# BadgerTechnologies/navigation

Measured on AMD Instinct MI355X. Metric: scored trajectories/sec (whole node) + costmap inflation cells/sec, 400x400 map, higher is better.
Workload: dtype f64

## Files before the change

### include/navgpu.h

```cpp
#ifndef NAVGPU_H_
#define NAVGPU_H_

#include <stddef.h>
#include <stdint.h>

#ifdef __cplusplus
extern "C" {
#endif

typedef enum {
  NAVGPU_OK = 0,
  NAVGPU_ERR_INVALID = -1,
  NAVGPU_ERR_NO_DEVICE = -2,
  NAVGPU_ERR_HIP = -3,
  NAVGPU_ERR_CAPACITY = -4,
  NAVGPU_ERR_STATE = -5
} navgpu_status;

#define NAVGPU_NO_INFORMATION 255
#define NAVGPU_LETHAL_OBSTACLE 254
#define NAVGPU_INSCRIBED_INFLATED_OBSTACLE 253
#define NAVGPU_FREE_SPACE 0

#define NAVGPU_LAYER_STATIC 1
// ... 177 lines not shown
  double acc_lim_x, acc_lim_y, acc_lim_theta;
  double xy_goal_tolerance, yaw_goal_tolerance;
  double trans_stopped_vel, rot_stopped_vel;
  int32_t prune_plan, reserved;
} navgpu_robot_limits;
int navgpu_planner_set_limits(navgpu_fleet* fleet, uint32_t first, uint32_t count, const navgpu_robot_limits* limits);
int navgpu_planner_get_limits(navgpu_fleet* fleet, uint32_t first, uint32_t count, navgpu_robot_limits* limits);
int navgpu_planner_set_plan(navgpu_fleet* fleet, uint32_t first, uint32_t count);
int navgpu_planner_stage(navgpu_fleet* fleet, uint32_t first, uint32_t count, const navgpu_robot_state* states,
                         const double* plan_xy, uint32_t n_plan_total);
int navgpu_planner_stage_poses(navgpu_fleet* fleet, uint32_t first, uint32_t count, const float* pos_xyth, const float* vel_xyth);
int navgpu_planner_cycle(navgpu_fleet* fleet, uint32_t first, uint32_t count);
int navgpu_planner_set_bounded_map_grids(navgpu_fleet* fleet, int32_t enable);
int navgpu_planner_set_seed_lists(navgpu_fleet* fleet, int32_t enable);
int navgpu_planner_set_split_prep(navgpu_fleet* fleet, int32_t enable);
int navgpu_planner_set_seed_list_capacity(navgpu_fleet* fleet, uint32_t cells);
int navgpu_planner_seed_list_counts(navgpu_fleet* fleet, uint32_t first, uint32_t count, uint32_t* counts);
int navgpu_planner_set_map_grid_options(navgpu_fleet* fleet, int32_t critic, int32_t aggregation, double yshift);
int navgpu_planner_wavefront_levels(navgpu_fleet* fleet, uint32_t first, uint32_t count, uint32_t* levels);
int navgpu_planner_wavefront_boxes(navgpu_fleet* fleet, uint32_t first, uint32_t count, int32_t* boxes);
int navgpu_planner_results(navgpu_fleet* fleet, uint32_t first, uint32_t count, navgpu_plan_result* results);
int navgpu_planner_set_cycles_in_flight(navgpu_fleet* fleet, int32_t cycles);
int navgpu_planner_results_previous(navgpu_fleet* fleet, uint32_t first, uint32_t count, navgpu_plan_result* results);
int navgpu_planner_trajectory(navgpu_fleet* fleet, uint32_t instance, double* xyth, uint32_t capacity_points);
int navgpu_planner_samples(navgpu_fleet* fleet, uint32_t instance, double* costs, int32_t* status,
                           float* velocities_xyz, uint32_t capacity);
int navgpu_planner_check_trajectory(navgpu_fleet* fleet, uint32_t instance, const float vel_samples[3], int32_t* ok);
int navgpu_planner_check_trajectories(navgpu_fleet* fleet, uint32_t n_robots, const uint32_t* instances,
                                      const uint32_t* probe_offsets , const float* vel_samples ,
                                      int32_t* ok , double* costs );
// ... 595 lines not shown
```

### navigation_amd/_lib.py

```python
import ctypes as C
import os
import subprocess

import numpy as np

_HERE = os.path.dirname(os.path.abspath(__file__))
_LIB = None

LAYER_STATIC, LAYER_OBSTACLE, LAYER_VOXEL, LAYER_INFLATION = 1, 2, 4, 8
GRID_MASTER, GRID_STATIC, GRID_OBSTACLE, GRID_VOXEL, GRID_PATH, GRID_GOAL, GRID_GOAL_FRONT = range(7)
OBS_MARKING, OBS_CLEARING = 1, 2
VOXEL_UNKNOWN, VOXEL_MARKED = 1, 2
K_OBSTACLE, K_MERGE, K_INFLATE, K_BFS, K_SCORE, K_SELECT, K_FOOTPRINT, K_VOXEL_EXPORT, K_OBS_INGEST, K_CHECK_TRAJ = range(10)
KERNELS = ("k_obstacle", "k_merge", "k_inflate", "k_bfs", "k_score", "k_select", "k_footprint_cost", "k_voxel_export", "k_obs_ingest", "k_check_traj")
CLOUD_XYZ, CLOUD_SCAN = 0, 1
OBSBUF_MAX_SOURCES, OBSBUF_MAX_CLOUD_POINTS = 8, 65536


class NavgpuError(RuntimeError):
    pass


class FleetDesc(C.Structure):
    _fields_ = [("n_instances", C.c_uint32), ("size_x", C.c_uint32), ("size_y", C.c_uint32),
# ... 439 lines not shown
    ("navgpu_costmap_update_list", C.c_int, [vp, u32, vp]),
    ("navgpu_costmap_bounds_list", C.c_int, [vp, u32, vp, vp]),
    ("navgpu_inflate", C.c_int, [vp, u32, u32, vp]),
    ("navgpu_obstacle_update_bounds", C.c_int, [vp, u32, u32, vp]),
    ("navgpu_obstacle_update_costs", C.c_int, [vp, u32, u32, vp]),
    ("navgpu_planner_configure", C.c_int, [vp, C.POINTER(DwaConfig)]),
    ("navgpu_planner_set_limits", C.c_int, [vp, C.c_uint32, C.c_uint32, vp]),
    ("navgpu_planner_get_limits", C.c_int, [vp, C.c_uint32, C.c_uint32, vp]),
    ("navgpu_planner_set_plan", C.c_int, [vp, u32, u32]),
    ("navgpu_planner_stage", C.c_int, [vp, u32, u32, vp, vp, u32]),
    ("navgpu_planner_stage_poses", C.c_int, [vp, u32, u32, vp, vp]),
    ("navgpu_planner_cycle", C.c_int, [vp, u32, u32]),
    ("navgpu_planner_set_bounded_map_grids", C.c_int, [vp, C.c_int32]),
    ("navgpu_planner_set_seed_lists", C.c_int, [vp, C.c_int32]),
    ("navgpu_planner_set_split_prep", C.c_int, [vp, C.c_int32]),
    ("navgpu_planner_set_seed_list_capacity", C.c_int, [vp, u32]),
    ("navgpu_planner_seed_list_counts", C.c_int, [vp, u32, u32, vp]),
    ("navgpu_planner_set_map_grid_options", C.c_int, [vp, C.c_int32, C.c_int32, C.c_double]),
    ("navgpu_planner_wavefront_levels", C.c_int, [vp, u32, u32, vp]),
    ("navgpu_planner_wavefront_boxes", C.c_int, [vp, u32, u32, vp]),
    ("navgpu_planner_results", C.c_int, [vp, u32, u32, vp]),
    ("navgpu_planner_set_cycles_in_flight", C.c_int, [vp, C.c_int32]),
    ("navgpu_planner_results_previous", C.c_int, [vp, u32, u32, vp]),
    ("navgpu_planner_trajectory", C.c_int, [vp, u32, vp, u32]),
    ("navgpu_planner_samples", C.c_int, [vp, u32, vp, vp, vp, u32]),
    ("navgpu_planner_check_trajectory", C.c_int, [vp, u32, vp, C.POINTER(i32)]),
    ("navgpu_planner_check_trajectories", C.c_int, [vp, u32, vp, vp, vp, vp, vp]),
    ("navgpu_planner_stage_list", C.c_int, [vp, u32, vp, vp, vp, u32]),
    ("navgpu_planner_stage_poses_list", C.c_int, [vp, u32, vp, vp, vp]),
    ("navgpu_planner_cycle_list", C.c_int, [vp, u32, vp]),
# ... 151 lines not shown
```

### navigation_amd/csrc/navgpu_device.h

```cpp
#pragma once
#include <hip/hip_runtime.h>
#include <stdint.h>

#include "../../include/navgpu.h"

namespace navgpu {

constexpr uint8_t kNoInfo = 255, kLethal = 254, kInscribed = 253, kFree = 0;
constexpr int kMaxFootprint = 32;
constexpr int kCareRows = 128, kCareWords = 4;
constexpr uint32_t kSeedListMax = 1024;
constexpr uint32_t kNoSeedList = 0xFFFFFFFFu;
#ifndef NAVGPU_SCORE_TAB_THREADS
#define NAVGPU_SCORE_TAB_THREADS 256
#endif
#ifndef NAVGPU_SCORE_TAB_LDS_KB
#define NAVGPU_SCORE_TAB_LDS_KB 14
#endif
#ifndef NAVGPU_SCORE_PREP_THREADS
#define NAVGPU_SCORE_PREP_THREADS 256
#endif
#ifndef NAVGPU_SCORE_THREADS
#define NAVGPU_SCORE_THREADS 256
#endif
// ... 111 lines not shown
  int32_t* axis_count;
  uint32_t *path, *goal, *goal_front;
  uint32_t* bfs_scratch;
  int32_t* bfs_box;
  uint32_t* bfs_care;
  uint32_t* bfs_reach;
  uint32_t bfs_bounded;
  unsigned long long* bfs_trace;
  uint32_t* bfs_next_item;
  uint32_t* bfs_free;
  uint32_t* bfs_levels;
  uint32_t* bfs_order;
  uint32_t* bfs_seed_cells;
  uint32_t* bfs_seed_count;
  uint32_t bfs_seed_cap;
  uint32_t bfs_grids;
  uint32_t* within;
  uint32_t win;
  uint32_t fp_rcells;
  uint8_t fp_halfw[32];
  uint32_t fp_chunk;
  uint32_t use_tables, tab_steps, tab_nfp, tab_nth;
  int32_t mg_agg[4];
  double mg_yshift[4];
  int32_t mg_generic;
  uint32_t tab_rows;
  uint32_t tab_bytes;
  double tab_dt;
  uint8_t* prep;
  uint32_t prep_stride, prep_bytes;
// ... 410 lines not shown
```

### navigation_amd/csrc/navgpu_fleet.h

```cpp
#pragma once
#include <algorithm>
#include <cfloat>
#include <cmath>
#include <cstdio>
#include <cstdlib>
#include <cstring>
#include <ctime>
#include <deque>
#include <mutex>
#include <string>
#include <vector>

#include "navgpu_device.h"

using namespace navgpu;

namespace navgpu {
extern thread_local std::string g_last_error;

#define HIP_TRY(expr)                                                                              \
  do {                                                                                             \
    hipError_t e_ = (expr);                                                                        \
    if (e_ != hipSuccess) {                                                                        \
      g_last_error = std::string(#expr) + ": " + hipGetErrorString(e_);                            \
// ... 45 lines not shown
  navgpu_inflation_params infl{};
  navgpu_obstacle_params obsp{};
  double fp_radius = 0.0;
  std::vector<void*> pinned;
  ObsCsr* hp_obs = nullptr;
  uint32_t *hp_cnt = nullptr, *hp_used = nullptr, *hp_plan_cnt = nullptr;
  float* hp_pts = nullptr;
  double *hp_fpw = nullptr, *hp_pose = nullptr, *hp_plan = nullptr, *hp_front = nullptr;
  int32_t *hp_shift = nullptr, *hp_align = nullptr;
  uint32_t *hp_reach = nullptr, *hp_fpn = nullptr;
  uint8_t *cm_stage_dev = nullptr, *cm_stage_host = nullptr, *pl_stage_dev = nullptr, *pl_stage_host = nullptr;
  size_t cm_stage_bytes = 0, pl_stage_bytes = 0;
  bool bounded_grids = true;
  bool seed_lists = true;
  bool split_prep = true;
  uint32_t seed_list_cap = kSeedListMax;
  std::vector<uint8_t> grid_partial;
  std::vector<int32_t> h_box;
  std::vector<uint64_t> inputs_gen, cycle_gen;
  void touchInputs(uint32_t first, uint32_t count) {
    for (uint32_t i = first; i < first + count && i < inputs_gen.size(); ++i) ++inputs_gen[i];
  }
  navgpu_robot_state* hp_state = nullptr;
  navgpu_plan_result* hp_result = nullptr;
  bool hp_dma_pending = false;
  int cycles_in_flight = 1;
  int res_slot = 0;
  hipEvent_t ev_cycle[2] = {nullptr, nullptr}, ev_cm_h2d = nullptr, ev_pl_h2d = nullptr;
  bool ev_cycle_set[2] = {false, false}, ev_cm_set = false, ev_pl_set = false;
  hipError_t waitMirrors(hipEvent_t ev, bool set) {
// ... 286 lines not shown
```

### navigation_amd/csrc/navgpu_host.cpp

```cpp
#include "navgpu_fleet.h"

namespace navgpu {
thread_local std::string g_last_error;
}

extern "C" {

const char* navgpu_version(void) { return "navgpu 0.1 (gfx950)"; }
const char* navgpu_strerror(int status) {
  switch (status) {
    case NAVGPU_OK: return "ok";
    case NAVGPU_ERR_INVALID: return "invalid argument";
    case NAVGPU_ERR_NO_DEVICE: return "no usable HIP device (this library has no CPU fallback)";
    case NAVGPU_ERR_HIP: return "HIP runtime error";
    case NAVGPU_ERR_CAPACITY: return "input exceeds a capacity given at fleet creation";
    case NAVGPU_ERR_STATE: return "call sequence violated";
    default: return "unknown status";
  }
}
const char* navgpu_last_error(void) { return g_last_error.c_str(); }
int navgpu_device_count(void) {
  int n = 0;
  if (hipGetDeviceCount(&n) != hipSuccess) return 0;
  return n;
// ... 184 lines not shown
  A(pl.goal, (size_t)n * pl.cells);
  A(pl.goal_front, (size_t)n * pl.cells);
  if (bfs_scratch_words(cm.nx, cm.ny)) A(pl.bfs_scratch, (size_t)n * bfs_scratch_words(cm.nx, cm.ny));
  pl.bfs_grids = 3;
  pl.within = nullptr;
  A(pl.bfs_box, (size_t)n * 8);
  A(pl.bfs_care, (size_t)n * kCareRows * kCareWords);
  A(pl.bfs_next_item, 4);
  A(pl.bfs_free, (size_t)n * cm.ny * ((cm.nx + 31) / 32));
  A(pl.bfs_levels, (size_t)n * 3);
  A(pl.bfs_order, (size_t)n * 3);
  A(pl.bfs_seed_cells, (size_t)n * 3 * kSeedListMax);
  A(pl.bfs_seed_count, (size_t)n * 3);
  pl.bfs_seed_cap = 0;
  pl.bfs_bounded = 0;
  A(pl.counters, (size_t)n * 2);
  A(pl.osc_flags, n);
  A(pl.osc_prev, (size_t)n * 3);
  A(pl.limits, n);
  A(pl.traj, (size_t)n * pl.max_sim_steps * 3);
#undef A
  f->h_origin.assign((size_t)n * 2, 0.0);
  f->h_fp_spec.assign((size_t)n * kMaxFootprint * 2, 0.0);
  f->h_fp_n.assign(n, 0);
  f->h_limits.assign(n, RobotLimits{});
  f->limits_dirty.assign(n, 0);
  f->lp_lim.assign(n, navgpu_local_limits{});
  f->grid_partial.assign(n, 0);
  f->obs_consumed.assign(n, 0);
  f->bounded_grids = true;
// ... 919 lines not shown
  if (!f) return NAVGPU_ERR_INVALID;
  FleetGuard guard_(f);
  f->bounded_grids = enable != 0;
  return restageReach(f);
}
int navgpu_planner_set_seed_lists(navgpu_fleet* f, int32_t enable) {
  if (!f) return NAVGPU_ERR_INVALID;
  FleetGuard guard_(f);
  f->seed_lists = enable != 0;
  return NAVGPU_OK;
}
int navgpu_planner_set_split_prep(navgpu_fleet* f, int32_t enable) {
  if (!f) return NAVGPU_ERR_INVALID;
  FleetGuard guard_(f);
  f->split_prep = enable != 0;
  return NAVGPU_OK;
}
static bool splitPrep(const navgpu_fleet* f) {
  return f->split_prep && split_prep_applies && launch_bfs_prep && launch_bfs_prep_list && launch_score_grids && launch_score_grids_list &&
         split_prep_applies(f->pl);
}
int navgpu_planner_set_seed_list_capacity(navgpu_fleet* f, uint32_t cells) {
  if (!f || cells == 0 || cells > kSeedListMax) return NAVGPU_ERR_INVALID;
  FleetGuard guard_(f);
  f->seed_list_cap = cells;
  return NAVGPU_OK;
}
int navgpu_planner_seed_list_counts(navgpu_fleet* f, uint32_t first, uint32_t count, uint32_t* counts) {
  if (!f || !counts || !f->rangeOk(first, count)) return NAVGPU_ERR_INVALID;
  FleetGuard guard_(f);
// ... 868 lines not shown
```

### navigation_amd/csrc/planner_bfs_rows.hip

```cpp
#include "planner_bfs_common.h"
#include "planner_score.h"

namespace navgpu {

#ifdef NAVGPU_BFS_STATS
__device__ unsigned long long g_bfs_stats[16];
#define BFS_STAMP(v) const unsigned long long v = __builtin_amdgcn_s_memtime()
#define BFS_ACC(i, x) bst[i] += (x)
#else
#define BFS_STAMP(v)
#define BFS_ACC(i, x)
#endif
#ifndef NAVGPU_ROWS_RECORD_PAD
#define NAVGPU_ROWS_RECORD_PAD 4
#endif
constexpr uint32_t kRowsRecordPad = NAVGPU_ROWS_RECORD_PAD;
template <int W>
__host__ __device__ inline size_t bfs_rows_lds_words(uint32_t nx, uint32_t ny) {
  constexpr uint32_t Wp = (W + 3) & ~3u;
  const uint32_t nw = bfs_rows_waves(ny);
  return (((size_t)nw * kRowsPerWave * ((nx + 31) >> 5) + 3) & ~(size_t)3) + (size_t)kCareRows * kCareWords + (size_t)(nw + 2) * 2 * kRowsHalo * (2 * Wp + kRowsRecordPad);
}
#define NAVGPU_ROWS_DPP " row_mask:0xf bank_mask:0xf bound_ctrl:1\n\t"
#define NAVGPU_ROWS_GROUP_WORDS                                    \
// ... 16 lines not shown
  "v_or_b32_dpp %[t1], %[f1], %[t1] wave_shl:1" NAVGPU_ROWS_DPP    \
  "v_or_b32_dpp %[t2], %[f2], %[t2] wave_shl:1" NAVGPU_ROWS_DPP    \
  "v_or_b32_dpp %[t3], %[f3], %[t3] wave_shl:1" NAVGPU_ROWS_DPP    \
  "v_bitop3_b32 %[f0], %[u0], %[b0], %[t0] bitop3:0x32\n\t"        \
  "v_bitop3_b32 %[f1], %[u1], %[b1], %[t1] bitop3:0x32\n\t"        \
  "v_bitop3_b32 %[f2], %[u2], %[b2], %[t2] bitop3:0x32\n\t"        \
  "v_bitop3_b32 %[f3], %[u3], %[b3], %[t3] bitop3:0x32\n\t"        \
  "v_or3_b32 %[b0], %[b0], %[u0], %[t0]\n\t"                       \
  "v_or3_b32 %[b1], %[b1], %[u1], %[t1]\n\t"                       \
  "v_or3_b32 %[b2], %[b2], %[u2], %[t2]\n\t"                       \
  "v_or3_b32 %[b3], %[b3], %[u3], %[t3]\n\t"
#define NAVGPU_ROWS_GROUP_REGS                                                                                                              \
  [b0] "+v"(b[0]), [b1] "+v"(b[1]), [b2] "+v"(b[2]), [b3] "+v"(b[3]), [f0] "+v"(f[0]), [f1] "+v"(f[1]), [f2] "+v"(f[2]), [f3] "+v"(f[3]), \
      [p] "=&v"(p), [u0] "=&v"(u0), [u1] "=&v"(u1), [u2] "=&v"(u2), [u3] "=&v"(u3), [t0] "=&v"(t0), [t1] "=&v"(t1), [t2] "=&v"(t2),       \
      [t3] "=&v"(t3)
__device__ __forceinline__ void rowsGroup4(const int g, const uint32_t aw, uint64_t& acc, uint32_t* __restrict__ b, uint32_t* __restrict__ f,
                                           const uint32_t L, const uint32_t R, uint32_t& p) {
  uint32_t u0, u1, u2, u3, t0, t1, t2, t3;
  uint64_t c0;
  asm volatile(NAVGPU_ROWS_GROUP_WORDS
               "v_or3_b32 %[u0], %[f0], %[f1], %[f2]\n\t"
               "v_or_b32_e32 %[u0], %[u0], %[f3]\n\t"
               "v_cmp_ne_u32_e64 %[c0], 0, %[u0]\n\t"
               "s_or_b64 %[acc], %[acc], %[c0]\n\t"
               "1:\n\t"
               : NAVGPU_ROWS_GROUP_REGS, [acc] "+s"(acc), [c0] "=&s"(c0)
               : [aw] "s"(aw), [g] "n"(g), [L] "v"(L), [R] "v"(R)
               : "scc");
}
__device__ __forceinline__ void rowsGroup4PerLevel(const int g, const uint32_t aw, uint32_t& nz, uint32_t& lo, uint32_t& hi, uint32_t* __restrict__ b,
                                                   uint32_t* __restrict__ f, const uint32_t L, const uint32_t R, uint32_t& p) {
  uint32_t u0, u1, u2, u3, t0, t1, t2, t3, st;
  uint64_t c0, c1, c2;
  asm volatile(NAVGPU_ROWS_GROUP_WORDS
               "v_or3_b32 %[u0], %[f0], %[f1], %[f2]\n\t"
               "v_cmp_ne_u32_e64 %[c1], 0, %[f0]\n\t"
               "v_or_b32_e32 %[u0], %[u0], %[f3]\n\t"
               "v_cmp_ne_u32_e64 %[c2], 0, %[f3]\n\t"
               "v_cmp_ne_u32_e64 %[c0], 0, %[u0]\n\t"
               "s_cmp_lg_u64 %[c1], 0\n\t"
               "s_cselect_b32 %[st], %[bit], 0\n\t"
               "s_or_b32 %[lo], %[lo], %[st]\n\t"
               "s_cmp_lg_u64 %[c2], 0\n\t"
               "s_cselect_b32 %[st], %[bit], 0\n\t"
// ... 81 lines not shown
  const bool wave_in_box = (int)(wave_id * kRowsPerWave) <= by1 && (int)((wave_id + 1) * kRowsPerWave) > by0;
  const bool row_in_box = owner && row_i >= by0 && row_i <= by1;
  const int w0 = rg.w0, w1 = rg.w1;
  const uint32_t region_groups = bfsRegionGroups(rg);
  uint32_t* drow = dist + (size_t)row * nx;
  auto storeCells = [&](int j, uint32_t cells, uint32_t value) { bfsStoreCells(drow + j * 32, cells, value, aligned4); };
  const bool pub_top = lane >= (uint32_t)D && lane < 2u * D, pub_bot = lane >= 64u - 2 * D && lane < 64u - D;
  const uint32_t pub_wr = (((wave_id + 1) * 2 + (pub_top ? 0u : 1u)) * D + (pub_top ? lane - D : lane - (64u - 2 * D))) * RS;
  const bool halo_top = lane < (uint32_t)D, halo_bot = lane >= 64u - D;
  const uint32_t halo_rd = ((halo_top ? (wave_id * 2 + 1) : ((wave_id + 2) * 2)) * D + (halo_top ? lane : lane - (64u - D))) * RS;
  constexpr uint32_t gmask = (1u << NG) - 1u;

  constexpr bool kBlockLive = W != 20;
  static_assert(D >= 1 && D < 32, "the edge masks take D bits of one word");
  constexpr uint32_t edge_lo = kBlockLive ? (1u << D) - 1u : 0xFFFFFFFFu, edge_hi = kBlockLive ? ~(0xFFFFFFFFu >> D) : 0xFFFFFFFFu;
  auto activity = [&]() -> uint32_t {
    uint32_t nz = 0, lo = 0, hi = 0;
#pragma unroll
    for (int q = 0; q < NG; ++q) {
      const uint32_t t = fr[4 * q] | fr[4 * q + 1] | fr[4 * q + 2] | fr[4 * q + 3];
      if (__builtin_amdgcn_ballot_w64(t != 0) != 0) {
        nz |= 1u << q;
        if (__builtin_amdgcn_ballot_w64((fr[4 * q] & edge_lo) != 0) != 0) lo |= 1u << q;
        if (__builtin_amdgcn_ballot_w64((fr[4 * q + 3] & edge_hi) != 0) != 0) hi |= 1u << q;
      }
    }
    return (nz | (lo >> 1) | (hi << 1)) & gmask;
  };
  if (wave_in_box) {
#pragma unroll
    for (int j = 0; j < W; ++j)
      if (j >= w0 && j <= w1 && row_in_box) storeCells(j, fr[j], 0u);
  }
  uint32_t a_own = activity();
  uint32_t level = 0, xch = 0;
  bfsStamp(pl, tid, item, 2);
  bool done = false;
#ifdef NAVGPU_BFS_STATS
  unsigned long long bst[9] = {0, 0, 0, 0, 0, 0, 0, 0, 0};
#endif
  auto storeNew = [&](const uint32_t groups) {
    if (wave_in_box && (groups & region_groups) != 0) {
#pragma unroll
      for (int q = 0; q < NG; ++q) {
        if (((groups & region_groups) >> q) & 1u) {
#pragma unroll
          for (int c = 0; c < 4; ++c) {
            const int j = 4 * q + c;
            if (j < W && j >= w0 && j <= w1) {
#ifndef NAVGPU_BFS_X_NOSTORE
              if (row_in_box && fr[j < W ? j : 0] != 0) storeCells(j, fr[j < W ? j : 0], level + 1);
#endif
            }
          }
        }
      }
    }
  };
  while (!done) {
    bool any_new;
    if constexpr (kBlockLive) {
      const uint32_t aw = __builtin_amdgcn_readfirstlane(a_own);
      uint64_t acc = 0;
      if (aw == 0) {
        BFS_ACC(5, D);
        level += D;
      } else {
        for (int k = 0; k < D; ++k) {
          BFS_STAMP(ts1);
          BFS_ACC(5, 1);
          BFS_ACC(7, 1);
          BFS_ACC(8, __builtin_popcount(aw));
          uint32_t awk = aw;
          asm volatile("" : "+s"(awk));
          uint32_t p[2];
          const uint32_t zero = 0;
#pragma unroll
          for (int q = 0; q < NG; ++q)
            rowsGroup4(q, awk, acc, &blocked[4 * q], &fr[4 * q], q > 0 ? p[(q + 1) & 1] : zero, q + 1 < NG ? fr[q + 1 < NG ? 4 * q + 4 : 0] : zero, p[q & 1]);
          BFS_STAMP(ts2);
          BFS_ACC(1, ts2 - ts1);
          storeNew(awk);
          BFS_STAMP(ts3);
          BFS_ACC(2, ts3 - ts2);
          ++level;
        }
      }
      any_new = acc != 0;
    } else {
      uint32_t any_blk = 0;
      for (int k = 0; k < D; ++k) {
        BFS_STAMP(ts1);
        BFS_ACC(5, 1);
        const uint32_t aw = __builtin_amdgcn_readfirstlane(a_own);
// ... 67 lines not shown
          blocked[q] = b.x;
          blocked[q + 1] = b.y;
          blocked[q + 2] = b.z;
          blocked[q + 3] = b.w;
        }
      }
      a_own = activity();
      __syncthreads();
    }
    ++xch;
    BFS_STAMP(ts6);
    BFS_ACC(4, ts6 - ts5);
  }
#ifdef NAVGPU_BFS_STATS
  if (lane == 0)
    for (int k = 0; k < 9; ++k) atomicAdd(&g_bfs_stats[k], bst[k]);
#endif
  bfsStamp(pl, tid, item, 3);

  __syncthreads();
  {
    uint32_t ex[WP], fb[WP];
#pragma unroll
    for (int j = 0; j < WP; ++j) {
      const bool in = owner && (uint32_t)j < Wr;
      fb[j] = in ? (freew[row * Wr + j] & ((uint32_t)j + 1 == Wr ? last_mask : 0xFFFFFFFFu)) : 0u;
      ex[j] = in ? ((blocked[j] & fb[j]) | seedm[row * Wr + j]) : 0u;
    }
    if (pub_top || pub_bot) {
#pragma unroll
      for (int j = 0; j < WP; ++j) edge[pub_wr + j] = ex[j];
// ... 275 lines not shown
    return (nz | (lo >> 1) | (hi << 1)) & gmask;
  };
  if (wave_in_box) {
#pragma unroll
    for (int j = 0; j < W; ++j)
      if (j >= w0 && j <= w1) {
        if (inA) storeCells(rowA, j, frA[j], 0u);
        if (inB) storeCells(rowB, j, frB[j], 0u);
      }
  }
  uint32_t a_own = activity();
  uint32_t level = 0, xch = 0;
  bfsStamp(pl, tid, item, 2);
  bool done = false;
#ifdef NAVGPU_BFS_STATS
  unsigned long long bst[9] = {0, 0, 0, 0, 0, 0, 0, 0, 0};
#endif
  while (!done) {
    const uint32_t aw = __builtin_amdgcn_readfirstlane(a_own);
    uint64_t acc = 0;
    for (int k = 0; k < D; ++k) {
      BFS_STAMP(ts1);
      BFS_ACC(5, 1);
      uint32_t awk = aw;
      asm volatile("" : "+s"(awk));
      BFS_ACC(7, awk != 0 ? 1 : 0);
      BFS_ACC(8, __builtin_popcount(awk));
      if (awk == 0) {
        ++level;
        continue;
      }
// ... 247 lines not shown
```

### navigation_amd/fleet.py

```python
import ctypes as C

import numpy as np

from . import _lib as N
from ._lib import (DwaConfig, FleetDesc, InflationParams, NavgpuError, Observation, ObstacleParams, PlanResult,
                   RobotState, check, lib)

_GRID_DTYPE = {N.GRID_MASTER: np.uint8, N.GRID_STATIC: np.uint8, N.GRID_OBSTACLE: np.uint8,
               N.GRID_VOXEL: np.uint32, N.GRID_PATH: np.uint32, N.GRID_GOAL: np.uint32,
               N.GRID_GOAL_FRONT: np.uint32}


def _ptr(a):
    return a.ctypes.data_as(C.c_void_p)


class Fleet:
    def __init__(self, n_instances, size_x, size_y, resolution, layers=N.LAYER_OBSTACLE | N.LAYER_INFLATION,
                 track_unknown=False, device=0, max_points=1024, max_observations=4, max_plan=256,
                 max_footprint=16, max_sim_steps=64, keep_sample_costs=False, rolling_window=False):
        self.L = lib()
        d = FleetDesc(n_instances, size_x, size_y, resolution, layers, int(track_unknown), device, max_points,
                      max_observations, max_plan, max_footprint, max_sim_steps, int(keep_sample_costs), int(rolling_window))
        self.desc = d
# ... 374 lines not shown
    AGGREGATIONS = {"last": 0, "sum": 1, "product": 2}

    def set_map_grid_options(self, critic, aggregation="last", yshift=0.0):
        check(self.L.navgpu_planner_set_map_grid_options(self.h, self.MAP_GRID_CRITICS[critic], self.AGGREGATIONS[aggregation], float(yshift)),
              "set_map_grid_options")

    def set_bounded_map_grids(self, enable):
        check(self.L.navgpu_planner_set_bounded_map_grids(self.h, 1 if enable else 0), "set_bounded_map_grids")

    def set_seed_lists(self, enable):
        check(self.L.navgpu_planner_set_seed_lists(self.h, 1 if enable else 0), "set_seed_lists")

    def set_split_prep(self, enable):
        check(self.L.navgpu_planner_set_split_prep(self.h, 1 if enable else 0), "set_split_prep")

    def set_seed_list_capacity(self, cells):
        check(self.L.navgpu_planner_set_seed_list_capacity(self.h, int(cells)), "set_seed_list_capacity")

    def seed_list_counts(self, first=0, count=None):
        first, count = self._range(first, count)
        out = np.zeros((count, 3), np.uint32)
        check(self.L.navgpu_planner_seed_list_counts(self.h, first, count, _ptr(out)), "seed_list_counts")
        return out

    def wavefront_levels(self, first=0, count=None):
        first, count = self._range(first, count)
        out = np.zeros((count, 3), np.uint32)
        check(self.L.navgpu_planner_wavefront_levels(self.h, first, count, _ptr(out)), "wavefront_levels")
        return out

# ... 450 lines not shown
```

Before: 6.867 billion.

## Restrict row-bitset BFS levels to a five-word live window per wave

Adds a word-window mode to the row-bitset BFS. When the activity mask is computed, each word is checked for frontier reach, and the start of a five-word window that covers every live word is encoded into the upper bits of the activity value. Each level then updates only those five words through hand-written inline assembly, and falls back to the per-group path when no window fits. This is meant to cut the ALU/DPP work per BFS level on sparse frontiers, at the price of an extra liveness scan per activity check and larger branchy asm blocks. It is enabled by default through a new fleet flag.

```diff
diff --git a/include/navgpu.h b/include/navgpu.h
--- a/include/navgpu.h
+++ b/include/navgpu.h
@@ -215,6 +215,7 @@
 int navgpu_planner_set_bounded_map_grids(navgpu_fleet* fleet, int32_t enable);
 int navgpu_planner_set_seed_lists(navgpu_fleet* fleet, int32_t enable);
 int navgpu_planner_set_split_prep(navgpu_fleet* fleet, int32_t enable);
+int navgpu_planner_set_bfs_word_window(navgpu_fleet* fleet, int32_t enable);
 int navgpu_planner_set_seed_list_capacity(navgpu_fleet* fleet, uint32_t cells);
 int navgpu_planner_seed_list_counts(navgpu_fleet* fleet, uint32_t first, uint32_t count, uint32_t* counts);
 int navgpu_planner_set_map_grid_options(navgpu_fleet* fleet, int32_t critic, int32_t aggregation, double yshift);
diff --git a/navigation_amd/_lib.py b/navigation_amd/_lib.py
--- a/navigation_amd/_lib.py
+++ b/navigation_amd/_lib.py
@@ -477,6 +477,7 @@
     ("navgpu_planner_set_bounded_map_grids", C.c_int, [vp, C.c_int32]),
     ("navgpu_planner_set_seed_lists", C.c_int, [vp, C.c_int32]),
     ("navgpu_planner_set_split_prep", C.c_int, [vp, C.c_int32]),
+    ("navgpu_planner_set_bfs_word_window", C.c_int, [vp, C.c_int32]),
     ("navgpu_planner_set_seed_list_capacity", C.c_int, [vp, u32]),
     ("navgpu_planner_seed_list_counts", C.c_int, [vp, u32, u32, vp]),
     ("navgpu_planner_set_map_grid_options", C.c_int, [vp, C.c_int32, C.c_int32, C.c_double]),
diff --git a/navigation_amd/csrc/navgpu_device.h b/navigation_amd/csrc/navgpu_device.h
--- a/navigation_amd/csrc/navgpu_device.h
+++ b/navigation_amd/csrc/navgpu_device.h
@@ -149,6 +149,7 @@
   uint32_t* bfs_seed_cells;
   uint32_t* bfs_seed_count;
   uint32_t bfs_seed_cap;
+  uint32_t bfs_word_window;
   uint32_t bfs_grids;
   uint32_t* within;
   uint32_t win;
diff --git a/navigation_amd/csrc/navgpu_fleet.h b/navigation_amd/csrc/navgpu_fleet.h
--- a/navigation_amd/csrc/navgpu_fleet.h
+++ b/navigation_amd/csrc/navgpu_fleet.h
@@ -83,6 +83,7 @@
   bool bounded_grids = true;
   bool seed_lists = true;
   bool split_prep = true;
+  bool bfs_word_window = true;
   uint32_t seed_list_cap = kSeedListMax;
   std::vector<uint8_t> grid_partial;
   std::vector<int32_t> h_box;
diff --git a/navigation_amd/csrc/navgpu_host.cpp b/navigation_amd/csrc/navgpu_host.cpp
--- a/navigation_amd/csrc/navgpu_host.cpp
+++ b/navigation_amd/csrc/navgpu_host.cpp
@@ -222,6 +222,7 @@
   A(pl.bfs_seed_count, (size_t)n * 3);
   pl.bfs_seed_cap = 0;
   pl.bfs_bounded = 0;
+  pl.bfs_word_window = f->bfs_word_window ? 1u : 0u;
   A(pl.counters, (size_t)n * 2);
   A(pl.osc_flags, n);
   A(pl.osc_prev, (size_t)n * 3);
@@ -1171,6 +1172,13 @@
   if (!f) return NAVGPU_ERR_INVALID;
   FleetGuard guard_(f);
   f->split_prep = enable != 0;
+  return NAVGPU_OK;
+}
+int navgpu_planner_set_bfs_word_window(navgpu_fleet* f, int32_t enable) {
+  if (!f) return NAVGPU_ERR_INVALID;
+  FleetGuard guard_(f);
+  f->bfs_word_window = enable != 0;
+  f->pl.bfs_word_window = enable != 0 ? 1u : 0u;
   return NAVGPU_OK;
 }
 static bool splitPrep(const navgpu_fleet* f) {
diff --git a/navigation_amd/csrc/planner_bfs_rows.hip b/navigation_amd/csrc/planner_bfs_rows.hip
--- a/navigation_amd/csrc/planner_bfs_rows.hip
+++ b/navigation_amd/csrc/planner_bfs_rows.hip
@@ -1,4 +1,5 @@
 #include "planner_bfs_common.h"
+#include "planner_bfs_window.h"
 #include "planner_score.h"
 
 namespace navgpu {
@@ -54,20 +55,225 @@
   [b0] "+v"(b[0]), [b1] "+v"(b[1]), [b2] "+v"(b[2]), [b3] "+v"(b[3]), [f0] "+v"(f[0]), [f1] "+v"(f[1]), [f2] "+v"(f[2]), [f3] "+v"(f[3]), \
       [p] "=&v"(p), [u0] "=&v"(u0), [u1] "=&v"(u1), [u2] "=&v"(u2), [u3] "=&v"(u3), [t0] "=&v"(t0), [t1] "=&v"(t1), [t2] "=&v"(t2),       \
       [t3] "=&v"(t3)
-__device__ __forceinline__ void rowsGroup4(const int g, const uint32_t aw, uint64_t& acc, uint32_t* __restrict__ b, uint32_t* __restrict__ f,
-                                           const uint32_t L, const uint32_t R, uint32_t& p) {
-  uint32_t u0, u1, u2, u3, t0, t1, t2, t3;
+#define NAVGPU_F(i) "%[f" #i "]"
+#define NAVGPU_B(i) "%[b" #i "]"
+#define NAVGPU_ROWS_LEVEL_WINDOW(Lw, a, b, c, d, e, Rw)                                                   \
+  "v_alignbit_b32 %[u0], " NAVGPU_F(a) ", " Lw ", 31\n\t"                                                 \
+  "v_alignbit_b32 %[u1], " NAVGPU_F(b) ", " NAVGPU_F(a) ", 31\n\t"                                        \
+  "v_alignbit_b32 %[u2], " NAVGPU_F(c) ", " NAVGPU_F(b) ", 31\n\t"                                        \
+  "v_alignbit_b32 %[u3], " NAVGPU_F(d) ", " NAVGPU_F(c) ", 31\n\t"                                        \
+  "v_alignbit_b32 %[u4], " NAVGPU_F(e) ", " NAVGPU_F(d) ", 31\n\t"                                        \
+  "v_alignbit_b32 %[t0], " NAVGPU_F(b) ", " NAVGPU_F(a) ", 1\n\t"                                         \
+  "v_alignbit_b32 %[t1], " NAVGPU_F(c) ", " NAVGPU_F(b) ", 1\n\t"                                         \
+  "v_alignbit_b32 %[t2], " NAVGPU_F(d) ", " NAVGPU_F(c) ", 1\n\t"                                         \
+  "v_alignbit_b32 %[t3], " NAVGPU_F(e) ", " NAVGPU_F(d) ", 1\n\t"                                         \
+  "v_alignbit_b32 %[t4], " Rw ", " NAVGPU_F(e) ", 1\n\t"                                                  \
+  "v_or_b32_dpp %[u0], " NAVGPU_F(a) ", %[u0] wave_shr:1" NAVGPU_ROWS_DPP                                 \
+  "v_or_b32_dpp %[u1], " NAVGPU_F(b) ", %[u1] wave_shr:1" NAVGPU_ROWS_DPP                                 \
+  "v_or_b32_dpp %[u2], " NAVGPU_F(c) ", %[u2] wave_shr:1" NAVGPU_ROWS_DPP                                 \
+  "v_or_b32_dpp %[u3], " NAVGPU_F(d) ", %[u3] wave_shr:1" NAVGPU_ROWS_DPP                                 \
+  "v_or_b32_dpp %[u4], " NAVGPU_F(e) ", %[u4] wave_shr:1" NAVGPU_ROWS_DPP                                 \
+  "v_or_b32_dpp %[t0], " NAVGPU_F(a) ", %[t0] wave_shl:1" NAVGPU_ROWS_DPP                                 \
+  "v_or_b32_dpp %[t1], " NAVGPU_F(b) ", %[t1] wave_shl:1" NAVGPU_ROWS_DPP                                 \
+  "v_or_b32_dpp %[t2], " NAVGPU_F(c) ", %[t2] wave_shl:1" NAVGPU_ROWS_DPP                                 \
+  "v_or_b32_dpp %[t3], " NAVGPU_F(d) ", %[t3] wave_shl:1" NAVGPU_ROWS_DPP                                 \
+  "v_or_b32_dpp %[t4], " NAVGPU_F(e) ", %[t4] wave_shl:1" NAVGPU_ROWS_DPP                                 \
+  "v_bitop3_b32 " NAVGPU_F(a) ", %[u0], " NAVGPU_B(a) ", %[t0] bitop3:0x32\n\t"                           \
+  "v_bitop3_b32 " NAVGPU_F(b) ", %[u1], " NAVGPU_B(b) ", %[t1] bitop3:0x32\n\t"                           \
+  "v_bitop3_b32 " NAVGPU_F(c) ", %[u2], " NAVGPU_B(c) ", %[t2] bitop3:0x32\n\t"                           \
+  "v_bitop3_b32 " NAVGPU_F(d) ", %[u3], " NAVGPU_B(d) ", %[t3] bitop3:0x32\n\t"                           \
+  "v_bitop3_b32 " NAVGPU_F(e) ", %[u4], " NAVGPU_B(e) ", %[t4] bitop3:0x32\n\t"                           \
+  "v_or3_b32 " NAVGPU_B(a) ", " NAVGPU_B(a) ", %[u0], %[t0]\n\t"                                          \
+  "v_or3_b32 " NAVGPU_B(b) ", " NAVGPU_B(b) ", %[u1], %[t1]\n\t"                                          \
+  "v_or3_b32 " NAVGPU_B(c) ", " NAVGPU_B(c) ", %[u2], %[t2]\n\t"                                          \
+  "v_or3_b32 " NAVGPU_B(d) ", " NAVGPU_B(d) ", %[u3], %[t3]\n\t"                                          \
+  "v_or3_b32 " NAVGPU_B(e) ", " NAVGPU_B(e) ", %[u4], %[t4]\n\t"                                          \
+  "v_or3_b32 %[u0], " NAVGPU_F(a) ", " NAVGPU_F(b) ", " NAVGPU_F(c) "\n\t"                                \
+  "v_or3_b32 %[u0], %[u0], " NAVGPU_F(d) ", " NAVGPU_F(e) "\n\t"                                          \
+  "v_cmp_ne_u32_e64 %[c0], 0, %[u0]\n\t"                                                                  \
+  "s_or_b64 %[acc], %[acc], %[c0]\n\t"
+#define NAVGPU_ROWS_LEVEL_GROUP(g, Lw, a, b, c, d, Rw, P)                                                 \
+  "v_mov_b32 " P ", " NAVGPU_F(d) "\n\t"                                                                  \
+  "s_bitcmp1_b32 %[aw], " #g "\n\t"                                                                       \
+  "s_cbranch_scc0 1f\n\t"                                                                                 \
+  "v_alignbit_b32 %[u0], " NAVGPU_F(a) ", " Lw ", 31\n\t"                                                 \
+  "v_alignbit_b32 %[u1], " NAVGPU_F(b) ", " NAVGPU_F(a) ", 31\n\t"                                        \
+  "v_alignbit_b32 %[u2], " NAVGPU_F(c) ", " NAVGPU_F(b) ", 31\n\t"                                        \
+  "v_alignbit_b32 %[u3], " NAVGPU_F(d) ", " NAVGPU_F(c) ", 31\n\t"                                        \
+  "v_alignbit_b32 %[t0], " NAVGPU_F(b) ", " NAVGPU_F(a) ", 1\n\t"                                         \
+  "v_alignbit_b32 %[t1], " NAVGPU_F(c) ", " NAVGPU_F(b) ", 1\n\t"                                         \
+  "v_alignbit_b32 %[t2], " NAVGPU_F(d) ", " NAVGPU_F(c) ", 1\n\t"                                         \
+  "v_alignbit_b32 %[t3], " Rw ", " NAVGPU_F(d) ", 1\n\t"                                                  \
+  "v_or_b32_dpp %[u0], " NAVGPU_F(a) ", %[u0] wave_shr:1" NAVGPU_ROWS_DPP                                 \
+  "v_or_b32_dpp %[u1], " NAVGPU_F(b) ", %[u1] wave_shr:1" NAVGPU_ROWS_DPP                                 \
+  "v_or_b32_dpp %[u2], " NAVGPU_F(c) ", %[u2] wave_shr:1" NAVGPU_ROWS_DPP                                 \
+  "v_or_b32_dpp %[u3], " NAVGPU_F(d) ", %[u3] wave_shr:1" NAVGPU_ROWS_DPP                                 \
+  "v_or_b32_dpp %[t0], " NAVGPU_F(a) ", %[t0] wave_shl:1" NAVGPU_ROWS_DPP                                 \
+  "v_or_b32_dpp %[t1], " NAVGPU_F(b) ", %[t1] wave_shl:1" NAVGPU_ROWS_DPP                                 \
+  "v_or_b32_dpp %[t2], " NAVGPU_F(c) ", %[t2] wave_shl:1" NAVGPU_ROWS_DPP                                 \
+  "v_or_b32_dpp %[t3], " NAVGPU_F(d) ", %[t3] wave_shl:1" NAVGPU_ROWS_DPP                                 \
+  "v_bitop3_b32 " NAVGPU_F(a) ", %[u0], " NAVGPU_B(a) ", %[t0] bitop3:0x32\n\t"                           \
+  "v_bitop3_b32 " NAVGPU_F(b) ", %[u1], " NAVGPU_B(b) ", %[t1] bitop3:0x32\n\t"                           \
+  "v_bitop3_b32 " NAVGPU_F(c) ", %[u2], " NAVGPU_B(c) ", %[t2] bitop3:0x32\n\t"                           \
+  "v_bitop3_b32 " NAVGPU_F(d) ", %[u3], " NAVGPU_B(d) ", %[t3] bitop3:0x32\n\t"                           \
+  "v_or3_b32 " NAVGPU_B(a) ", " NAVGPU_B(a) ", %[u0], %[t0]\n\t"                                          \
+  "v_or3_b32 " NAVGPU_B(b) ", " NAVGPU_B(b) ", %[u1], %[t1]\n\t"                                          \
+  "v_or3_b32 " NAVGPU_B(c) ", " NAVGPU_B(c) ", %[u2], %[t2]\n\t"                                          \
+  "v_or3_b32 " NAVGPU_B(d) ", " NAVGPU_B(d) ", %[u3], %[t3]\n\t"                                          \
+  "v_or3_b32 %[u0], " NAVGPU_F(a) ", " NAVGPU_F(b) ", " NAVGPU_F(c) "\n\t"                                \
+  "v_or_b32_e32 %[u0], %[u0], " NAVGPU_F(d) "\n\t"                                                        \
+  "v_cmp_ne_u32_e64 %[c0], 0, %[u0]\n\t"                                                                  \
+  "s_or_b64 %[acc], %[acc], %[c0]\n\t"                                                                    \
+  "1:\n\t"
+#define NAVGPU_ROWS_LEVEL_REGS8                                                                                                             \
+  [b0] "+v"(b[0]), [b1] "+v"(b[1]), [b2] "+v"(b[2]), [b3] "+v"(b[3]), [b4] "+v"(b[4]), [b5] "+v"(b[5]), [b6] "+v"(b[6]), [b7] "+v"(b[7]), \
+      [f0] "+v"(f[0]), [f1] "+v"(f[1]), [f2] "+v"(f[2]), [f3] "+v"(f[3]), [f4] "+v"(f[4]), [f5] "+v"(f[5]), [f6] "+v"(f[6]), [f7] "+v"(f[7])
+#define NAVGPU_ROWS_LEVEL_REGS16                                                                                                                     \
+  NAVGPU_ROWS_LEVEL_REGS8, [b8] "+v"(b[8]), [b9] "+v"(b[9]), [b10] "+v"(b[10]), [b11] "+v"(b[11]), [b12] "+v"(b[12]), [b13] "+v"(b[13]),             \
+      [b14] "+v"(b[14]), [b15] "+v"(b[15]), [f8] "+v"(f[8]), [f9] "+v"(f[9]), [f10] "+v"(f[10]), [f11] "+v"(f[11]), [f12] "+v"(f[12]), [f13] "+v"(f[13]), \
+      [f14] "+v"(f[14]), [f15] "+v"(f[15])
+#define NAVGPU_ROWS_LEVEL_TEMPS                                                                                                              \
+  [u0] "=&v"(u0), [u1] "=&v"(u1), [u2] "=&v"(u2), [u3] "=&v"(u3), [u4] "=&v"(u4), [t0] "=&v"(t0), [t1] "=&v"(t1), [t2] "=&v"(t2), [t3] "=&v"(t3), \
+      [t4] "=&v"(t4), [acc] "+s"(acc), [c0] "=&s"(c0)
+static_assert(kRowsWindow == 5, "NAVGPU_ROWS_LEVEL_WINDOW is written out for five words");
+template <int W>
+__device__ __forceinline__ void rowsLevel(const uint32_t aw, uint64_t& acc, uint32_t* __restrict__ b, uint32_t* __restrict__ f) {
+  static_assert(W == 7 || W == 13, "one statement per row size, its words and windows written out");
+  uint32_t u0, u1, u2, u3, u4, t0, t1, t2, t3, t4;
   uint64_t c0;
-  asm volatile(NAVGPU_ROWS_GROUP_WORDS
-               "v_or3_b32 %[u0], %[f0], %[f1], %[f2]\n\t"
-               "v_or_b32_e32 %[u0], %[u0], %[f3]\n\t"
-               "v_cmp_ne_u32_e64 %[c0], 0, %[u0]\n\t"
-               "s_or_b64 %[acc], %[acc], %[c0]\n\t"
-               "1:\n\t"
-               : NAVGPU_ROWS_GROUP_REGS, [acc] "+s"(acc), [c0] "=&s"(c0)
-               : [aw] "s"(aw), [g] "n"(g), [L] "v"(L), [R] "v"(R)
-               : "scc");
-}
+  if constexpr (W == 7) {
+    asm volatile("s_bitcmp1_b32 %[aw], 9\n\t"
+                 "s_cbranch_scc1 12f\n\t"
+                 "s_bitcmp1_b32 %[aw], 8\n\t"
+                 "s_cbranch_scc0 20f\n\t"
+                 NAVGPU_ROWS_LEVEL_WINDOW(NAVGPU_F(0), 1, 2, 3, 4, 5, NAVGPU_F(6))
+                 "s_branch 9f\n\t"
+                 "20:\n\t"
+                 NAVGPU_ROWS_LEVEL_WINDOW("0", 0, 1, 2, 3, 4, NAVGPU_F(5))
+                 "s_branch 9f\n\t"
+                 "12:\n\t"
+                 "s_bitcmp1_b32 %[aw], 8\n\t"
+                 "s_cbranch_scc0 22f\n\t"
+                 NAVGPU_ROWS_LEVEL_GROUP(0, "0", 0, 1, 2, 3, NAVGPU_F(4), "%[u4]")
+                 NAVGPU_ROWS_LEVEL_GROUP(1, "%[u4]", 4, 5, 6, 7, "0", "%[t4]")
+                 "s_branch 9f\n\t"
+                 "22:\n\t"
+                 NAVGPU_ROWS_LEVEL_WINDOW(NAVGPU_F(1), 2, 3, 4, 5, 6, NAVGPU_F(7))
+                 "9:\n\t"
+                 : NAVGPU_ROWS_LEVEL_REGS8, NAVGPU_ROWS_LEVEL_TEMPS
+                 : [aw] "s"(aw)
+                 : "scc");
+  } else {
+    asm volatile("s_bitcmp1_b32 %[aw], 11\n\t"
+                 "s_cbranch_scc1 18f\n\t"
+                 "s_bitcmp1_b32 %[aw], 10\n\t"
+                 "s_cbranch_scc1 14f\n\t"
+                 "s_bitcmp1_b32 %[aw], 9\n\t"
+                 "s_cbranch_scc1 12f\n\t"
+                 "s_bitcmp1_b32 %[aw], 8\n\t"
+                 "s_cbranch_scc0 20f\n\t"
+                 NAVGPU_ROWS_LEVEL_WINDOW(NAVGPU_F(0), 1, 2, 3, 4, 5, NAVGPU_F(6))
+                 "s_branch 9f\n\t"
+                 "20:\n\t"
+                 NAVGPU_ROWS_LEVEL_WINDOW("0", 0, 1, 2, 3, 4, NAVGPU_F(5))
+                 "s_branch 9f\n\t"
+                 "12:\n\t"
+                 "s_bitcmp1_b32 %[aw], 8\n\t"
+                 "s_cbranch_scc0 22f\n\t"
+                 NAVGPU_ROWS_LEVEL_WINDOW(NAVGPU_F(2), 3, 4, 5, 6, 7, NAVGPU_F(8))
+                 "s_branch 9f\n\t"
+                 "22:\n\t"
+                 NAVGPU_ROWS_LEVEL_WINDOW(NAVGPU_F(1), 2, 3, 4, 5, 6, NAVGPU_F(7))
+                 "s_branch 9f\n\t"
+                 "14:\n\t"
+                 "s_bitcmp1_b32 %[aw], 9\n\t"
+                 "s_cbranch_scc1 16f\n\t"
+                 "s_bitcmp1_b32 %[aw], 8\n\t"
+                 "s_cbranch_scc0 24f\n\t"
+                 NAVGPU_ROWS_LEVEL_WINDOW(NAVGPU_F(4), 5, 6, 7, 8, 9, NAVGPU_F(10))
+                 "s_branch 9f\n\t"
+                 "24:\n\t"
+                 NAVGPU_ROWS_LEVEL_WINDOW(NAVGPU_F(3), 4, 5, 6, 7, 8, NAVGPU_F(9))
+                 "s_branch 9f\n\t"
+                 "16:\n\t"
+                 "s_bitcmp1_b32 %[aw], 8\n\t"
+                 "s_cbranch_scc0 26f\n\t"
+                 NAVGPU_ROWS_LEVEL_WINDOW(NAVGPU_F(6), 7, 8, 9, 10, 11, NAVGPU_F(12))
+                 "s_branch 9f\n\t"
+                 "26:\n\t"
+                 NAVGPU_ROWS_LEVEL_WINDOW(NAVGPU_F(5), 6, 7, 8, 9, 10, NAVGPU_F(11))
+                 "s_branch 9f\n\t"
+                 "18:\n\t"
+                 "s_bitcmp1_b32 %[aw], 10\n\t"
+                 "s_cbranch_scc0 28f\n\t"
+                 NAVGPU_ROWS_LEVEL_GROUP(0, "0", 0, 1, 2, 3, NAVGPU_F(4), "%[u4]")
+                 NAVGPU_ROWS_LEVEL_GROUP(1, "%[u4]", 4, 5, 6, 7, NAVGPU_F(8), "%[t4]")
+                 NAVGPU_ROWS_LEVEL_GROUP(2, "%[t4]", 8, 9, 10, 11, NAVGPU_F(12), "%[u4]")
+                 NAVGPU_ROWS_LEVEL_GROUP(3, "%[u4]", 12, 13, 14, 15, "0", "%[t4]")
+                 "s_branch 9f\n\t"
+                 "28:\n\t"
+                 NAVGPU_ROWS_LEVEL_WINDOW(NAVGPU_F(7), 8, 9, 10, 11, 12, NAVGPU_F(13))
+                 "9:\n\t"
+                 : NAVGPU_ROWS_LEVEL_REGS16, NAVGPU_ROWS_LEVEL_TEMPS
+                 : [aw] "s"(aw)
+                 : "scc");
+  }
+}
+#define NAVGPU_ROWS_WORD_LIVE(Lw, w, Rw)            \
+  "v_and_b32_e32 %[t], %[lo], " Rw "\n\t"           \
+  "v_and_or_b32 %[t], " Lw ", %[hi], %[t]\n\t"      \
+  "v_or_b32_e32 %[t], %[t], " w "\n\t"              \
+  "v_cmp_ne_u32_e64 %[c], 0, %[t]\n\t"              \
+  "s_cmp_lg_u64 %[c], 0\n\t"                        \
+  "s_addc_u32 %[live], %[live], %[live]\n\t"
+#define NAVGPU_ROWS_GROUP_LIVE(g, Lw, a, b, c, d, Rw)                 \
+  "s_lshl_b32 %[st], %[live], 4\n\t"                                  \
+  "s_bitcmp1_b32 %[a], " #g "\n\t"                                    \
+  "s_cbranch_scc0 1f\n\t"                                             \
+  NAVGPU_ROWS_WORD_LIVE(NAVGPU_F(c), NAVGPU_F(d), Rw)                 \
+  NAVGPU_ROWS_WORD_LIVE(NAVGPU_F(b), NAVGPU_F(c), NAVGPU_F(d))        \
+  NAVGPU_ROWS_WORD_LIVE(NAVGPU_F(a), NAVGPU_F(b), NAVGPU_F(c))        \
+  NAVGPU_ROWS_WORD_LIVE(Lw, NAVGPU_F(a), NAVGPU_F(b))                 \
+  "s_mov_b32 %[st], %[live]\n\t"                                      \
+  "1:\n\t"                                                            \
+  "s_mov_b32 %[live], %[st]\n\t"
+#define NAVGPU_ROWS_LIVE_IN8 \
+  [f0] "v"(f[0]), [f1] "v"(f[1]), [f2] "v"(f[2]), [f3] "v"(f[3]), [f4] "v"(f[4]), [f5] "v"(f[5]), [f6] "v"(f[6]), [f7] "v"(f[7])
+#define NAVGPU_ROWS_LIVE_IN16 \
+  NAVGPU_ROWS_LIVE_IN8, [f8] "v"(f[8]), [f9] "v"(f[9]), [f10] "v"(f[10]), [f11] "v"(f[11]), [f12] "v"(f[12]), [f13] "v"(f[13]), [f14] "v"(f[14]), [f15] "v"(f[15])
+template <int W>
+__device__ __forceinline__ uint32_t rowsLiveWords(const uint32_t a, const uint32_t* __restrict__ f, const uint32_t lo, const uint32_t hi) {
+  static_assert(W == 7 || W == 13, "one statement per row size");
+  uint32_t live = 0, st, t;
+  uint64_t c;
+  if constexpr (W == 7) {
+    asm volatile(NAVGPU_ROWS_GROUP_LIVE(1, NAVGPU_F(3), 4, 5, 6, 7, NAVGPU_F(7))
+                 NAVGPU_ROWS_GROUP_LIVE(0, "0", 0, 1, 2, 3, NAVGPU_F(4))
+                 : [live] "+s"(live), [st] "=&s"(st), [t] "=&v"(t), [c] "=&s"(c)
+                 : NAVGPU_ROWS_LIVE_IN8, [a] "s"(a), [lo] "s"(lo), [hi] "s"(hi)
+                 : "scc");
+  } else {
+    asm volatile(NAVGPU_ROWS_GROUP_LIVE(3, NAVGPU_F(11), 12, 13, 14, 15, NAVGPU_F(15))
+                 NAVGPU_ROWS_GROUP_LIVE(2, NAVGPU_F(7), 8, 9, 10, 11, NAVGPU_F(12))
+                 NAVGPU_ROWS_GROUP_LIVE(1, NAVGPU_F(3), 4, 5, 6, 7, NAVGPU_F(8))
+                 NAVGPU_ROWS_GROUP_LIVE(0, "0", 0, 1, 2, 3, NAVGPU_F(4))
+                 : [live] "+s"(live), [st] "=&s"(st), [t] "=&v"(t), [c] "=&s"(c)
+                 : NAVGPU_ROWS_LIVE_IN16, [a] "s"(a), [lo] "s"(lo), [hi] "s"(hi)
+                 : "scc");
+  }
+  return live & ((1u << W) - 1u);
+}
+#undef NAVGPU_ROWS_LIVE_IN16
+#undef NAVGPU_ROWS_LIVE_IN8
+#undef NAVGPU_ROWS_GROUP_LIVE
+#undef NAVGPU_ROWS_WORD_LIVE
+#undef NAVGPU_ROWS_LEVEL_TEMPS
+#undef NAVGPU_ROWS_LEVEL_REGS16
+#undef NAVGPU_ROWS_LEVEL_REGS8
+#undef NAVGPU_ROWS_LEVEL_GROUP
+#undef NAVGPU_ROWS_LEVEL_WINDOW
+#undef NAVGPU_B
+#undef NAVGPU_F
 __device__ __forceinline__ void rowsGroup4PerLevel(const int g, const uint32_t aw, uint32_t& nz, uint32_t& lo, uint32_t& hi, uint32_t* __restrict__ b,
                                                    uint32_t* __restrict__ f, const uint32_t L, const uint32_t R, uint32_t& p) {
   uint32_t u0, u1, u2, u3, t0, t1, t2, t3, st;
@@ -179,6 +385,9 @@
   constexpr bool kBlockLive = W != 20;
   static_assert(D >= 1 && D < 32, "the edge masks take D bits of one word");
   constexpr uint32_t edge_lo = kBlockLive ? (1u << D) - 1u : 0xFFFFFFFFu, edge_hi = kBlockLive ? ~(0xFFFFFFFFu >> D) : 0xFFFFFFFFu;
+  const bool word_window = kBlockLive && pl.bfs_word_window != 0;
+  constexpr int kRowsWindowShift = 8;
+  static_assert(!kBlockLive || (kRowsNoWindow == 15 && W - kRowsWindow < 12), "rowsLevel tells a window's first word from kRowsNoWindow by four bits of the mask");
   auto activity = [&]() -> uint32_t {
     uint32_t nz = 0, lo = 0, hi = 0;
 #pragma unroll
@@ -190,7 +399,13 @@
         if (__builtin_amdgcn_ballot_w64((fr[4 * q + 3] & edge_hi) != 0) != 0) hi |= 1u << q;
       }
     }
-    return (nz | (lo >> 1) | (hi << 1)) & gmask;
+    const uint32_t a = (nz | (lo >> 1) | (hi << 1)) & gmask;
+    if constexpr (kBlockLive) {
+      uint32_t live = 0;
+      if (word_window && a != 0) live = rowsLiveWords<W>(a, fr, edge_lo, edge_hi);
+      return a | (uint32_t)bfsWindowStart(live, W, kRowsWindow) << kRowsWindowShift;
+    }
+    return a;
   };
   if (wave_in_box) {
 #pragma unroll
@@ -202,7 +417,7 @@
   bfsStamp(pl, tid, item, 2);
   bool done = false;
 #ifdef NAVGPU_BFS_STATS
-  unsigned long long bst[9] = {0, 0, 0, 0, 0, 0, 0, 0, 0};
+  unsigned long long bst[11] = {0, 0, 0, 0, 0, 0, 0, 0, 0, 0, 0};
 #endif
   auto storeNew = [&](const uint32_t groups) {
     if (wave_in_box && (groups & region_groups) != 0) {
@@ -227,22 +442,19 @@
     if constexpr (kBlockLive) {
       const uint32_t aw = __builtin_amdgcn_readfirstlane(a_own);
       uint64_t acc = 0;
-      if (aw == 0) {
+      if ((aw & gmask) == 0) {
         BFS_ACC(5, D);
         level += D;
       } else {
+        BFS_ACC((aw >> kRowsWindowShift) != (uint32_t)kRowsNoWindow ? 9 : 10, 1);
         for (int k = 0; k < D; ++k) {
           BFS_STAMP(ts1);
           BFS_ACC(5, 1);
           BFS_ACC(7, 1);
-          BFS_ACC(8, __builtin_popcount(aw));
+          BFS_ACC(8, __builtin_popcount(aw & gmask));
           uint32_t awk = aw;
           asm volatile("" : "+s"(awk));
-          uint32_t p[2];
-          const uint32_t zero = 0;
-#pragma unroll
-          for (int q = 0; q < NG; ++q)
-            rowsGroup4(q, awk, acc, &blocked[4 * q], &fr[4 * q], q > 0 ? p[(q + 1) & 1] : zero, q + 1 < NG ? fr[q + 1 < NG ? 4 * q + 4 : 0] : zero, p[q & 1]);
+          rowsLevel<W>(awk, acc, blocked, fr);
           BFS_STAMP(ts2);
           BFS_ACC(1, ts2 - ts1);
           storeNew(awk);
@@ -340,7 +552,7 @@
   }
 #ifdef NAVGPU_BFS_STATS
   if (lane == 0)
-    for (int k = 0; k < 9; ++k) atomicAdd(&g_bfs_stats[k], bst[k]);
+    for (int k = 0; k < 11; ++k) atomicAdd(&g_bfs_stats[k], bst[k]);
 #endif
   bfsStamp(pl, tid, item, 3);
 
@@ -646,7 +858,7 @@
   bfsStamp(pl, tid, item, 2);
   bool done = false;
 #ifdef NAVGPU_BFS_STATS
-  unsigned long long bst[9] = {0, 0, 0, 0, 0, 0, 0, 0, 0};
+  unsigned long long bst[11] = {0, 0, 0, 0, 0, 0, 0, 0, 0, 0, 0};
 #endif
   while (!done) {
     const uint32_t aw = __builtin_amdgcn_readfirstlane(a_own);
diff --git a/navigation_amd/csrc/planner_bfs_window.h b/navigation_amd/csrc/planner_bfs_window.h
--- /dev/null
+++ b/navigation_amd/csrc/planner_bfs_window.h
@@ -0,0 +1,29 @@
+#pragma once
+#include <stdint.h>
+
+#if defined(__HIPCC__) || defined(__CUDACC__)
+#define NAVGPU_WINDOW_FN __host__ __device__ inline
+#else
+#define NAVGPU_WINDOW_FN inline
+#endif
+
+namespace navgpu {
+
+constexpr int kRowsWindow = 5;
+constexpr int kRowsNoWindow = 15;
+
+NAVGPU_WINDOW_FN uint32_t bfsWordReach(uint32_t word, uint32_t left, uint32_t right, int halo) {
+  const uint32_t edge_lo = (1u << halo) - 1u, edge_hi = ~(0xFFFFFFFFu >> halo);
+  return word | (right & edge_lo) | (left & edge_hi);
+}
+NAVGPU_WINDOW_FN uint32_t bfsLiveWords(uint32_t nz, uint32_t lo, uint32_t hi, int words) {
+  return (nz | (lo >> 1) | (hi << 1)) & ((1u << words) - 1u);
+}
+NAVGPU_WINDOW_FN int bfsWindowStart(uint32_t live, int words, int window) {
+  if (live == 0 || words < window || (live >> words) != 0) return kRowsNoWindow;
+  const int first = __builtin_ctz(live);
+  const int s = first < words - window ? first : words - window;
+  return (live >> (s + window)) != 0 ? kRowsNoWindow : s;
+}
+
+}
diff --git a/navigation_amd/fleet.py b/navigation_amd/fleet.py
--- a/navigation_amd/fleet.py
+++ b/navigation_amd/fleet.py
@@ -412,6 +412,9 @@
     def set_split_prep(self, enable):
         check(self.L.navgpu_planner_set_split_prep(self.h, 1 if enable else 0), "set_split_prep")
 
+    def set_bfs_word_window(self, enable):
+        check(self.L.navgpu_planner_set_bfs_word_window(self.h, 1 if enable else 0), "set_bfs_word_window")
+
     def set_seed_list_capacity(self, cells):
         check(self.L.navgpu_planner_set_seed_list_capacity(self.h, int(cells)), "set_seed_list_capacity")
 
```

Result: no change. 6.881 billion (median of 5 runs) (+0.2%).
